# aehogan/lammps-induced-dipole-polarization-pair-style

Measured on AMD Instinct MI355X. Metric: atom-steps/sec, higher is better.
Workload: dtype f64

## Files before the change

### lammps-induced-dipole-polarization-pair-style_amd/csrc/polar_api.hip

```cpp
#include "polar_handle.hpp"

namespace {
void upload_types(polar_handle *h, int ntypes, const double *const t[7]) {
  need_device(h);
  const size_t m = (size_t)(ntypes + 1) * (ntypes + 1);
  std::vector<double> pack(8 * m, 0.0);
  for (size_t k = 0; k < m; k++) {
    pack[8 * k + 0] = t[6][k]; pack[8 * k + 1] = t[5][k]; pack[8 * k + 2] = t[0][k]; pack[8 * k + 3] = t[1][k];
    pack[8 * k + 4] = t[2][k]; pack[8 * k + 5] = t[3][k]; pack[8 * k + 6] = t[4][k];
  }
  h->d_lj.ensure(8 * m);
  HIPCHECK(hipMemcpy(h->d_lj.p, pack.data(), 8 * m * sizeof(double), hipMemcpyHostToDevice));
  h->P.ntypes = ntypes;
  h->P.ljpack = h->d_lj.p;
  h->ntypes = ntypes;
  h->types_set = true;
}

void upload_coul(polar_handle *h, double g_ewald, double qqrd2e, const double *slj, const double *scoul, int nbits,
                 int mask, int shift, double tabinnersq, const double *const t[8]) {
  need_device(h);
  h->P.g_ewald = g_ewald; h->P.qqrd2e = qqrd2e;
  for (int k = 0; k < 4; k++) { h->P.special_lj[k] = slj[k]; h->P.special_coul[k] = scoul[k]; }
  h->P.ncoultablebits = nbits; h->P.ncoulmask = mask; h->P.ncoulshiftbits = shift; h->P.tabinnersq = tabinnersq;
// ... 141 lines not shown
  int n = polar_device_count();
  if (n <= 0 || device < 0 || device >= n) {
    h->have_device = false;
    h->err = "no usable HIP device";
    return POLAR_OK;
  }
  return guarded(h, [&]() {
    HIPCHECK(hipSetDevice(device));
    HIPCHECK(hipStreamCreate(&h->stream));
    for (auto &e : h->ev) HIPCHECK(hipEventCreate(&e));
    {
      int prio_lo = 0, prio_hi = 0;
      HIPCHECK(hipDeviceGetStreamPriorityRange(&prio_lo, &prio_hi));
      HIPCHECK(hipStreamCreateWithPriority(&h->lj_stream, hipStreamNonBlocking, prio_lo));
    }
    HIPCHECK(hipEventCreate(&h->ev_fork)); HIPCHECK(hipEventCreate(&h->ev_join));
    HIPCHECK(hipEventCreate(&h->ev_lj0)); HIPCHECK(hipEventCreate(&h->ev_lj1));
    HIPCHECK(hipEventCreateWithFlags(&h->ev_dl0, hipEventDisableTiming)); HIPCHECK(hipEventCreateWithFlags(&h->ev_dl1, hipEventDisableTiming));
    HIPCHECK(hipEventCreateWithFlags(&h->ev_mu_ready, hipEventDisableTiming));
    for (auto &e : h->ev_fchunk) HIPCHECK(hipEventCreateWithFlags(&e, hipEventDisableTiming));
    for (auto &e : h->ev_ks) HIPCHECK(hipEventCreate(&e));
    HIPCHECK(hipStreamCreateWithFlags(&h->dl_stream, hipStreamNonBlocking));
    if (getenv("POLAR_NO_OVERLAP")) h->overlap_lj = false;
    if (const char *e = getenv("POLAR_LJ_PERS")) h->lj_pers = atoi(e);
    if (const char *e = getenv("POLAR_LJ_PERS_THREADS")) h->lj_pers_threads = std::max(256, std::min(POLAR_LJ_PERS_THREADS, (atoi(e) / 64) * 64));
    { int ncu = 0; if (hipDeviceGetAttribute(&ncu, hipDeviceAttributeMultiprocessorCount, device) == hipSuccess) h->ncu = ncu; }
    HIPCHECK(hipHostMalloc((void **)&h->h_scal, sizeof(Scal)));
    HIPCHECK(hipHostMalloc((void **)&h->h_flags, 16 * sizeof(int)));
    HIPCHECK(hipHostMalloc((void **)&h->h_ddtot, 64 * 16 * sizeof(unsigned long long)));
    h->d_overflow.ensure(16); h->d_ddtot.ensure(64 * 16);
    h->d_scal.ensure(1);
    h->d_slots.ensure((size_t)POLAR_NSLOT * POLAR_SLOT_STRIDE);
    h->have_device = true;
    return POLAR_OK;
  });
}

int polar_destroy(polar_handle *h) {
  if (!h) return POLAR_OK;
  if (h->have_device) {
    (void)hipSetDevice(h->device);
    (void)hipStreamSynchronize(h->stream);
    if (h->lj_stream) { (void)hipStreamSynchronize(h->lj_stream); (void)hipStreamDestroy(h->lj_stream); }
    for (hipEvent_t e : {h->ev_fork, h->ev_join, h->ev_lj0, h->ev_lj1, h->ev_dl0, h->ev_dl1, h->ev_mu_ready}) if (e) (void)hipEventDestroy(e);
    for (hipEvent_t e : h->ev_ks) if (e) (void)hipEventDestroy(e);
    if (h->dl_stream) (void)hipStreamDestroy(h->dl_stream);
// ... 817 lines not shown
```

### lammps-induced-dipole-polarization-pair-style_amd/csrc/polar_handle.hpp

```cpp
#pragma once
#include <hip/hip_runtime.h>

#include <algorithm>
#include <initializer_list>
#include <utility>
#include <chrono>
#include <cmath>
#include <cstdio>
#include <cstdlib>
#include <exception>
#include <cstring>
#include <numeric>
#include <string>
#include <thread>
#include <mutex>
#include <condition_variable>
#include <functional>
#include <memory>
#include <stdexcept>
#include <unistd.h>
#include <vector>

#include "pair_host.hpp"
#include "polar_kernels.hpp"
// ... 225 lines not shown
  int un_pitch = 0;
  int un_lds = 0;
  long long pitch16 = 0;
  int tile_max_u = 0;
  bool tile_reported = false;
  double dens = 0.0;
  std::vector<TileLaunch> tile_launches;
  TileLaunch tile_all{};
  size_t tile_lds_attr[16] = {0, 0, 0, 0, 0, 0, 0, 0, 0, 0, 0, 0, 0, 0, 0, 0};
  size_t tile_build_lds_attr = 0;
  int tile_waves = 4;
  int tile_wide = 0;
  int tile_sw[3] = {2, 2, 2};
  int deterministic = 0;
  Scal *h_scal = nullptr;
  hipEvent_t ev[8] = {};
  hipStream_t lj_stream = nullptr;
  hipEvent_t ev_fork = nullptr, ev_join = nullptr, ev_lj0 = nullptr, ev_lj1 = nullptr, ev_dl0 = nullptr, ev_dl1 = nullptr;
  hipStream_t dl_stream = nullptr;
  hipEvent_t ev_mu_ready = nullptr;
  double *early_mu = nullptr, *early_ef = nullptr, *user_mu = nullptr, *user_ef = nullptr;
  hipEvent_t ev_fchunk[4] = {nullptr, nullptr, nullptr, nullptr};
  bool overlap_lj = true;
  bool lj_forked = false;
  std::vector<double> h_tmp;
  double *h_stage = nullptr;
  DBuf<double> d_trace;
  DBuf<double4> d_ew_kv; DBuf<int4> d_ew_hkl, d_ew_rows;
  DBuf<double2> d_ew_s, d_ew_m, d_ew_part;
  DBuf<double> d_ew_erec, d_ew_vpart, d_ew_out;
  std::vector<double> ew_key;
  int ew_nk = 0, ew_nrow = 0, ew_nm = 0;
  double ew_cell[6] = {0, 0, 0, 0, 0, 0};
  hipEvent_t ev_ks[4] = {nullptr, nullptr, nullptr, nullptr};
  int ntrace = 0;
  size_t h_stage_cap = 0;
};
inline int fail(polar_handle *h, int code, const std::string &m) {
  if (h) h->err = m;
  return code;
}

template <typename F>
int guarded(polar_handle *h, F &&fn) {
  if (!h) return POLAR_ERR_STATE;
  try {
// ... 123 lines not shown
inline bool look_at_state(const polar_handle *h, int sw, int every, int step = 1) {
  const int done_sweeps = sw + 1;
  const int pred = h->last_sweeps;
  if (pred <= 0) return (sw % every) == every - 1;
  if (done_sweeps < pred) return (done_sweeps % 16) == 0;
  const int past = done_sweeps - pred;
  if (past <= 4 * step) return (past % step) == 0;
  return (past % every) == 0;
}
inline bool tile_mode(const polar_handle *h) { return h->ph.st.dd_cutoff > 0.0 && h->sweep_kernel == 4; }
inline MuView mu_view(const polar_handle *h) {
  if (tile_mode(h)) return MuView{reinterpret_cast<char *>(h->d_srec0.p), reinterpret_cast<char *>(h->d_srec1.p), (int)sizeof(SRec)};
  return MuView{reinterpret_cast<char *>(h->d_rec0.p), reinterpret_cast<char *>(h->d_rec1.p), (int)sizeof(AtomRec)};
}
inline const int *own_rows(const polar_handle *h) { return (h->sorted && sharded(h)) ? h->d_ownrows.p : nullptr; }

struct TileUnavailable : std::runtime_error {
  explicit TileUnavailable(const std::string &m) : std::runtime_error(m) {}
};

void launch_scan(long long n, const int *in, long long *out, DBuf<long long> &tot, hipStream_t s);
void build_cells(polar_handle *h);
void compute_slots(polar_handle *h);
void build_lists(polar_handle *h);
void launch_rank_pass(polar_handle *h, bool allpairs, int pass);
void prepare_lp(polar_handle *h);
void sweep_once(polar_handle *h, bool ap);
void sweep_phase(polar_handle *h, int color, int part);
void read_scal(polar_handle *h);
void debug_trace(polar_handle *h, int sw, bool jacobi);
bool accel_begin(polar_handle *h, bool ap);
void accel_export(polar_handle *h, double *dev_local_dots);
void accel_step(polar_handle *h, const double *global_dots);
void accel_export_fused(polar_handle *h, double *ared);
void accel_decide_mix(polar_handle *h, const double *ared, bool diff_first);
void solve(polar_handle *h, bool ap, polar_result *out);
void phase_begin(polar_handle *h, int eflag, int vflag, const double *mu_host);
int phase_finish(polar_handle *h, polar_result *out);
void clear_flags(polar_handle *h);
void tile_fallback(polar_handle *h);
bool grow_pitches(polar_handle *h);
int do_compute(polar_handle *h, int eflag, int vflag, const double *mu_host, polar_result *out);
void step_begin_lists(polar_handle *h, int eflag, int vflag);
bool step_needs_colors(const polar_handle *h);
void step_begin_finish(polar_handle *h);
void build_cluster_lists(polar_handle *h);
void ensure_colors(polar_handle *h);
// ... 9 lines not shown
```

### lammps-induced-dipole-polarization-pair-style_amd/csrc/polar_lists.hpp

```cpp
#pragma once

#include "polar_common.hpp"

namespace polar {

struct CellGrid {
  int trim;
  int nc[3];
  double lo[3], inv[3];
};

__device__ __forceinline__ int cell_of(const CellGrid &g, const Box &b, double x, double y, double z) {
  int c[3];
  double fr3[3];
  frac_coords(b, g.lo, x, y, z, fr3);
#pragma unroll
  for (int k = 0; k < 3; k++) {
    double fr = fr3[k];
    fr -= floor(fr);
    int ck = (int)(fr * g.nc[k]);
    c[k] = ck >= g.nc[k] ? g.nc[k] - 1 : ck;
  }
  return (c[2] * g.nc[1] + c[1]) * g.nc[0] + c[0];
}

// ... 423 lines not shown
                                  const int *__restrict__ sub, int nsub) {
  const long long c = blockIdx.x * (long long)blockDim.x + threadIdx.x;
  if (c >= ncell) return;
  const int a = (int)cell_first[c], e = a + npol[c];
  for (int q = 0; q < nclass; q++) {
    int k = 0;
    for (int j = a; j < e; j++) k += color_class(j, color_s, perm, own_lo, own_hi, sub, nsub) == q;
    cnt[(size_t)q * ncell + c] = k;
  }
}
static __global__ void k_color_fill(long long ncell, int nclass, const long long *__restrict__ cell_first, const int *__restrict__ npol,
                             const int *__restrict__ color_s, const int *__restrict__ perm, const long long *__restrict__ off,
                             int *__restrict__ rows_orig, int own_lo, int own_hi, const int *__restrict__ sub, int nsub) {
  const long long c = blockIdx.x * (long long)blockDim.x + threadIdx.x;
  if (c >= ncell) return;
  const int a = (int)cell_first[c], e = a + npol[c];
  for (int q = 0; q < nclass; q++) {
    long long w = off[(size_t)q * ncell + c];
    for (int j = a; j < e; j++) if (color_class(j, color_s, perm, own_lo, own_hi, sub, nsub) == q) rows_orig[w++] = perm[j];
  }
}

template <bool TRI, bool RECHECK>
static __global__ __launch_bounds__(POLAR_BLOCK) void k_nl_build(const int *__restrict__ rows, int nrows,
                                                          const double4 *__restrict__ pos4, Box box, CellGrid g,
                                                          const long long *__restrict__ cell_first, double cutallsq,
                                                          double ddcutsq, long long nl_pitch, long long dd_pitch,
                                                          int *__restrict__ nl_cnt, int *__restrict__ dd_cnt,
                                                          int *__restrict__ nl_j, int *__restrict__ dd_j,
                                                          double *__restrict__ dd_r2, int pad_dd,
                                                          int dd_shift_qm, int dd_pad_index, int *__restrict__ dd_wrap,
                                                          const int *__restrict__ color_s, double colordistsq,
                                                          int *__restrict__ color_conflict,
                                                          const int *__restrict__ dd_slot,
                                                          int *__restrict__ overflow,
                                                          unsigned long long *__restrict__ dd_total) {
  const int dd_shift = dd_shift_qm & 255, dd_qm = dd_shift_qm >> 8;
  const int lane = threadIdx.x & 63;
  const int row = blockIdx.x * POLAR_ROWS_PER_BLOCK + (threadIdx.x >> 6);
  if (row >= nrows) return;
  const int i = rows ? rows[row] : row;
  const double4 ri = pos4[i];
  const int imol = __double2hiint(ri.w), ipol = __double2loint(ri.w);
  const int icol = (RECHECK && color_s && ipol) ? color_s[i] : -2;
  bool clash = RECHECK && color_s && ipol && icol < 0;
  int cc[3];
  double uu[3], edge[3];
  {
    double fr3[3];
    frac_coords(box, g.lo, ri.x, ri.y, ri.z, fr3);
#pragma unroll
    for (int k = 0; k < 3; k++) {
      double fr = fr3[k];
      fr -= floor(fr);
      const double t = fr * g.nc[k];
      int ck = (int)t;
      ck = ck >= g.nc[k] ? g.nc[k] - 1 : ck;
      cc[k] = __builtin_amdgcn_readfirstlane(ck);
      uu[k] = wave_uniform(t - ck); edge[k] = wave_uniform(box.prd[k] / g.nc[k]);
    }
  }
  const int c0 = cc[0], c1 = cc[1], c2 = cc[2];
  const int slot_i = dd_slot ? dd_slot[i] : i;
// ... 65 lines not shown
          if (dd_r2) dd_r2[dd0 + kd] = rsq;
        }
        ncount += __popcll(m_nl);
        dcount += __popcll(m_dd);
      }
    }
  }
  if (pad_dd) {
    const int have = dcount < dd_pitch ? dcount : (int)dd_pitch;
    const int padded = (have + 63) & ~63;
    for (int k = have + lane; k < padded; k += 64) {
      dd_j[dd0 + (dd_shift ? lp_slot(k, dd_qm) : (long long)k)] = (dd_pad_index >= 0 ? dd_pad_index : i) << dd_shift;
      if (dd_r2) dd_r2[dd0 + k] = 1e60;
    }
  }
  if (RECHECK && color_s && __ballot(clash) != 0ull && lane == 0) atomicOr(color_conflict, 1);
  const unsigned long long anywrap = __ballot(wrap_lane);
  if (lane == 0) {
    nl_cnt[i] = ncount; dd_cnt[i] = dcount;
    if (dd_wrap) dd_wrap[i] = anywrap != 0ull;
    if (ncount > nl_pitch || dcount > dd_pitch) atomicMax(overflow, ncount > dcount ? ncount : dcount);
    if (dcount) atomicAdd(dd_total + (blockIdx.x & 63) * 16, (unsigned long long)(dcount < dd_pitch ? dcount : (int)dd_pitch));
  }
}

#ifdef POLAR_LAB
#include "lab/lists_paired_rows.hpp"
#endif

#ifdef POLAR_LAB
#include "lab/lists_cluster_rows.hpp"
#endif

struct LJGrid {
  int nc[3];
  double lo[3], inv[3];
};
__device__ __forceinline__ int lj_cell_of(const LJGrid &g, double x, double y, double z) {
  const double p[3] = {x, y, z};
  int c[3];
#pragma unroll
  for (int k = 0; k < 3; k++) {
    int ck = (int)floor((p[k] - g.lo[k]) * g.inv[k]);
    c[k] = ck < 0 ? 0 : (ck >= g.nc[k] ? g.nc[k] - 1 : ck);
  }
  return (c[2] * g.nc[1] + c[1]) * g.nc[0] + c[0];
// ... 227 lines not shown
```

### lammps-induced-dipole-polarization-pair-style_amd/csrc/polar_rows.hpp

```cpp
#pragma once

#include "polar_common.hpp"
#include "polar_force_pair.hpp"
#ifdef POLAR_LAB
#include "lab/force_pair_literal.hpp"
#define POLAR_LIT_PARAM , int literal
#define POLAR_LIT_PASS , literal
#else
#define POLAR_LIT_PARAM
#define POLAR_LIT_PASS
#endif

namespace polar {

static __global__ void k_pack(int n, const int *__restrict__ perm, const double *__restrict__ x, const double *__restrict__ q,
                       const double *__restrict__ alpha, const int *__restrict__ mol, const double *__restrict__ mu0,
                       AtomRec *__restrict__ r0, AtomRec *__restrict__ r1, int *__restrict__ mol_s,
                       double4 *__restrict__ pos4, double4 *__restrict__ xq_s, int wrap, Box box, double lo0, double lo1,
                       double lo2) {
  int i = blockIdx.x * blockDim.x + threadIdx.x;
  if (i == n) {
    AtomRec d;
    d.x = n > 0 ? x[0] : 0.0; d.y = n > 0 ? x[1] : 0.0; d.z = n > 0 ? x[2] : 0.0;
    d.mx = d.my = d.mz = d.q = d.a = 0.0;
// ... 337 lines not shown
  double4 *ctab_lds = reinterpret_cast<double4 *>(lj_lds + nlj);
  for (int t = threadIdx.x; t < w * w * 8; t += blockDim.x) lj_lds[t] = P.ljpack[t];
  const int ntable = 1 << P.ncoultablebits;
  for (int b = threadIdx.x; b < ntable; b += blockDim.x) {
    const double2 *bin = reinterpret_cast<const double2 *>(P.ctab + (size_t)b * 8);
    const double2 fdf = bin[1], ede = bin[2];
    ctab_lds[b] = make_double4(fdf.x, fdf.y, ede.x, ede.y);
  }
  __syncthreads();
  const int lane = threadIdx.x & 63, wv = threadIdx.x >> 6, nwv = blockDim.x >> 6;
  double ev = 0.0, ec = 0.0;
  for (int ii = blockIdx.x + gridDim.x * wv; ii < inum; ii += gridDim.x * nwv) {
    const int i = ilist ? ilist[ii] : ii;
    const int jnum = numneigh ? numneigh[i] : (int)(first[i + 1] - first[i]);
    if (jnum == 0) continue;
    double v[6] = {0, 0, 0, 0, 0, 0};
    ljcoul_row<EFLAG, VPAIR, TAB>(P, i, jnum, neigh + first[i], xq[i], xq, type, lj_lds, ctab_lds, lane, f, eatom, vatom, ev, ec, v);
    if (VPAIR) ljcoul_tally<false, true>(slots, ii, lane, vglobal, 0.0, 0.0, v);
  }
  const double none[6] = {0, 0, 0, 0, 0, 0};
  ljcoul_tally<EFLAG, false>(slots, blockIdx.x * nwv + wv, lane, 0, ev, ec, none);
}

template <bool ALLPAIRS, bool EW>
static __device__ __forceinline__ void static_field_body(const int *__restrict__ rows, int nrows, int nlocal,
                                                              const AtomRec *__restrict__ rec,
                                                              const int *__restrict__ mol, Box box,
                                                              RowList nl,
                                                              const int *__restrict__ nl_j, double cut_coulsq,
                                                              double e2s, double gamma, int use_previous,
                                                              double *__restrict__ ef, AtomRec *__restrict__ rec0,
                                                              AtomRec *__restrict__ rec1, const double4 *__restrict__ xq_s,
                                                              double g_ewald, const double *__restrict__ erec) {
  const int lane = threadIdx.x & 63;
  const int row = blockIdx.x * POLAR_ROWS_PER_BLOCK + (threadIdx.x >> 6);
  if (row >= nrows) return;
  const int i = rows ? rows[row] : row;
  const AtomRec ri = uniform_rec(rec[i]);
  const int mi = mol[i];
  const double f_shift = -1.0 / cut_coulsq;
  double ex = 0, ey = 0, ez = 0;
  long long beg = 0, end = nlocal;
  if (!ALLPAIRS) row_range(nl, i, beg, end);
  if (ALLPAIRS) {
    for (long long p = beg + lane; p < end; p += 64) {
      const int j = (int)p;
      if (j == i) continue;
      const AtomRec rj = rec[j];
      double dx, dy, dz;
      pair_del<ALLPAIRS>(box, ri.x, ri.y, ri.z, rj.x, rj.y, rj.z, dx, dy, dz);
      const double rsq = dx * dx + dy * dy + dz * dz;
      if (EW) {
        if (rsq <= cut_coulsq) {
          const double ef_temp = ewald_b1(rsq, g_ewald, (mi != mol[j]) || mi == 0) * rj.q;
          ex += ef_temp * dx; ey += ef_temp * dy; ez += ef_temp * dz;
        }
      } else if (rsq <= cut_coulsq && ((mi != mol[j]) || mi == 0)) {
        const double rinv = rsqrt(rsq);
        const double ef_temp = (rinv * rinv + f_shift) * rinv * rj.q;
        ex += ef_temp * dx; ey += ef_temp * dy; ez += ef_temp * dz;
      }
    }
  } else {
    __shared__ double2 s_stage[POLAR_ROWS_PER_BLOCK][64 * 5];
    double2 *stage = s_stage[threadIdx.x >> 6];
    for (long long base = beg; base < end; base += 64) {
      const long long p = base + lane;
      const bool valid = p < end;
      const int e = valid ? nl_j[p] : i;
      const int j = e & POLAR_NL_MASK;
      double xj, yj, zj, qj;
      if (xq_s) { const XQ t = fetch_xq(xq_s, j, stage, lane); xj = t.a.x; yj = t.a.y; zj = t.b.x; qj = t.b.y; }
      else { const RecQuad rj = fetch_records(rec, j, stage, lane); xj = rj.a.x; yj = rj.b.x; zj = rj.c.x; qj = rj.d.x; }
      double dx, dy, dz;
      pair_del<ALLPAIRS>(box, ri.x, ri.y, ri.z, xj, yj, zj, dx, dy, dz);
      const double rsq = dx * dx + dy * dy + dz * dz;
      if (EW) {
        if (valid && j != i && rsq <= cut_coulsq) {
          const double ef_temp = ewald_b1(rsq, g_ewald, !(e & POLAR_NL_SAMEMOL)) * qj;
          ex += ef_temp * dx; ey += ef_temp * dy; ez += ef_temp * dz;
        }
      } else if (valid && j != i && rsq <= cut_coulsq && !(e & POLAR_NL_SAMEMOL)) {
        const double rinv = rsqrt(rsq);
        const double ef_temp = (rinv * rinv + f_shift) * rinv * qj;
        ex += ef_temp * dx; ey += ef_temp * dy; ez += ef_temp * dz;
      }
    }
  }
  ex = wave_sum(ex); ey = wave_sum(ey); ez = wave_sum(ez);
  if (lane == 0) {
    ex *= e2s; ey *= e2s; ez *= e2s;
    if (EW) { ex += erec[3 * i]; ey += erec[3 * i + 1]; ez += erec[3 * i + 2]; }
    ef[3 * i] = ex; ef[3 * i + 1] = ey; ef[3 * i + 2] = ez;
    if (!use_previous) {
      const double a = ri.a;
      double mx = a * ex, my = a * ey, mz = a * ez;
      mx *= gamma; my *= gamma; mz *= gamma;
      rec0[i].mx = mx; rec0[i].my = my; rec0[i].mz = mz;
      rec1[i].mx = mx; rec1[i].my = my; rec1[i].mz = mz;
    }
  }
}

template <bool ALLPAIRS>
static __global__ __launch_bounds__(POLAR_BLOCK) void k_static_field(const int *__restrict__ rows, int nrows, int nlocal,
                                                              const AtomRec *__restrict__ rec,
                                                              const int *__restrict__ mol, Box box,
                                                              RowList nl,
                                                              const int *__restrict__ nl_j, double cut_coulsq,
                                                              double e2s, double gamma, int use_previous,
                                                              double *__restrict__ ef, AtomRec *__restrict__ rec0,
                                                              AtomRec *__restrict__ rec1, const double4 *__restrict__ xq_s) {
  static_field_body<ALLPAIRS, false>(rows, nrows, nlocal, rec, mol, box, nl, nl_j, cut_coulsq, e2s, gamma, use_previous, ef, rec0, rec1,
                                     xq_s, 0.0, nullptr);
}
template <bool ALLPAIRS>
static __global__ __launch_bounds__(POLAR_BLOCK) void k_ew_static_field(const int *__restrict__ rows, int nrows, int nlocal,
                                                                 const AtomRec *__restrict__ rec,
                                                                 const int *__restrict__ mol, Box box,
                                                                 RowList nl,
                                                                 const int *__restrict__ nl_j, double cut_coulsq,
                                                                 double e2s, double gamma, int use_previous,
                                                                 double *__restrict__ ef, AtomRec *__restrict__ rec0,
                                                                 AtomRec *__restrict__ rec1, const double4 *__restrict__ xq_s,
// ... 160 lines not shown
```

### lammps-induced-dipole-polarization-pair-style_amd/csrc/polar_step.hip

```cpp
#include "polar_handle.hpp"

void launch_scan(long long n, const int *in, long long *out, DBuf<long long> &tot, hipStream_t s) {
  const int nb = (int)std::max<long long>(1, (n + POLAR_SCAN_ITEMS - 1) / POLAR_SCAN_ITEMS);
  tot.ensure((size_t)nb + 1);
  k_scan_block<<<nb, 1024, 0, s>>>(n, in, out, tot.p);
  if (nb > 1) {
    k_scan_totals<<<1, 1024, 0, s>>>(nb, tot.p, out + n);
    k_scan_add<<<nblk(n - POLAR_SCAN_ITEMS, 256), 256, 0, s>>>(n, out, tot.p);
  }
}

void build_cells(polar_handle *h) {
  const polar_settings &st = h->ph.st;
  const int n = h->nlocal;
  const double cutall = std::max(st.cut_coul, st.dd_cutoff);
  double width[3];
  box_widths(h->box, width);
  for (int k = 0; k < 3; k++)
    if (h->box.periodic[k] && width[k] < 2.0 * cutall * (1.0 - 1e-12))
      throw InputError("dd_cutoff mode needs box lengths >= 2*max(cut_coul,dd_cutoff); use exact mode (dd_cutoff 0)");
  CellGrid &g = h->grid;
  g.trim = 1;
#ifdef POLAR_LAB
  if (const char *e = getenv("POLAR_NL_TRIM")) g.trim = atoi(e);
// ... 46 lines not shown
    h->d_ownrows.ensure(own_n(h) + 1);
    k_map_range<<<nblk(own_n(h), 256), 256, 0, s>>>(own_lo(h), own_n(h), h->d_inv.p, h->d_ownrows.p);
  }
}

void compute_slots(polar_handle *h) {
  const polar_settings &st = h->ph.st;
  const bool gs = st.polar_gs || st.polar_gs_ranked;
  const int n = h->nlocal;
  hipStream_t s = h->stream;
  h->d_slot.ensure(n + 1);
  HIPCHECK(hipMemsetAsync(h->d_slot.p, 0xFF, (size_t)(n + 1) * sizeof(int), s));
  if (gs && h->colors_valid) {
    const int tot = h->color_off.empty() ? 0 : h->color_off.back();
    if (tot > 0) k_slot_from_rows<<<nblk(tot, 256), 256, 0, s>>>(tot, h->d_rows.p, h->d_slot.p);
    h->slots_by_color = true;
    h->slots_epoch = h->color_epoch;
  } else {
    k_slot_from_rows<<<nblk(own_n(h), 256), 256, 0, s>>>(own_n(h), own_rows(h), h->d_slot.p);
    h->slots_by_color = false;
  }
}

void build_lists(polar_handle *h) {
  const polar_settings &st = h->ph.st;
  const int n = h->nlocal;
  const double cutall = std::max(st.cut_coul, st.dd_cutoff);
  hipStream_t s = h->stream;
  const CellGrid &g = h->grid;
  if (h->nl_pitch == 0 && getenv("POLAR_INIT_PITCH")) h->nl_pitch = h->dd_pitch = ((std::max(64, atoi(getenv("POLAR_INIT_PITCH"))) + 63) / 64) * 64;
  if (h->nl_pitch == 0) {
    double vol = h->box.prd[0] * h->box.prd[1] * h->box.prd[2];
    {
      int nc[3];
      long long tot = 1;
      for (int k = 0; k < 3; k++) { nc[k] = std::max(1, std::min(64, (int)(h->box.prd[k] / cutall))); tot *= nc[k]; }
      std::vector<char> occ((size_t)tot, 0);
      for (int a = 0; a < n; a++) {
        long long c = 0, mul = 1;
        for (int k = 0; k < 3; k++) {
          double fr = (h->hx[3 * (size_t)a + k] - h->grid.lo[k]) / h->box.prd[k];
          fr -= std::floor(fr);
          c += mul * std::min(nc[k] - 1, (int)(fr * nc[k]));
          mul *= nc[k];
        }
        occ[(size_t)c] = 1;
      }
// ... 23 lines not shown
  h->stream_mode = mode;
  const bool r2c = mode == 1;
  if (mode == 1) h->d_dd_r2.ensure((size_t)n * h->dd_pitch + 64);
  else if (mode == 0) h->d_dd_s.ensure((size_t)n * h->dd_pitch + 64);
  double *r2p = r2c ? h->d_dd_r2.p : nullptr;
  double2 *sp = mode == 0 ? h->d_dd_s.p : nullptr;
  bool fuse = mode != 0 && mode != 4;
#ifdef POLAR_LAB
  if (getenv("POLAR_NO_FUSE_R2")) fuse = false;
#endif
  const double cutallsq = cutall * cutall, ddsq = mode == 4 ? -1.0 : st.dd_cutoff * st.dd_cutoff;
  const int nr = own_n(h);
  const int *rows = own_rows(h);
  zero_many(s, {{h->d_nl_cnt.p, (size_t)(n + 1) * sizeof(int)}, {h->d_dd_cnt.p, (size_t)(n + 1) * sizeof(int)},
                {h->d_overflow.p, 16 * sizeof(int)}, {h->d_ddtot.p, 64 * 16 * sizeof(unsigned long long)}});
  const bool lp = mode == 3;
  if (lp) h->d_dd_wrap.ensure(n + 1);
  const bool recheck = h->colors_valid && h->colors_recheck && h->sweep_kernel < 3 && (int)h->h_color.size() == n;
  if (h->colors_recheck && !recheck) { h->colors_valid = false; h->colors_recheck = false; }
  if (recheck) {
    h->d_color_s.ensure(n + 1);
    k_color_map<<<nblk(n, 256), 256, 0, s>>>(n, h->d_perm.p, h->d_color_orig.p, h->d_color_s.p);
  }
#define NLB(TRI, RC)                                                                                                          \
  k_nl_build<TRI, RC><<<nblk(nr, POLAR_ROWS_PER_BLOCK), POLAR_BLOCK, 0, s>>>(                                                 \
      rows, nr, h->d_pos4.p, h->box, g, h->d_cell_first.p, cutallsq, ddsq, h->nl_pitch, h->dd_pitch, h->d_nl_cnt.p,            \
      h->d_dd_cnt.p, h->d_nl_j.p, h->d_dd_j.p, fuse ? r2p : nullptr, fuse ? 1 : 0, lp ? (6 | (h->lp_quad_major << 8)) : 0,    \
      lp ? n : -1, lp ? h->d_dd_wrap.p : nullptr, recheck ? h->d_color_s.p : nullptr, h->color_keep * h->color_keep,           \
      h->d_overflow.p + 8, lp ? h->d_slot.p : nullptr, h->d_overflow.p, h->d_ddtot.p)
  if (h->box.triclinic) { if (recheck) NLB(true, true); else NLB(true, false); }
  else                  { if (recheck) NLB(false, true); else NLB(false, false); }
#undef NLB
  const RowList ddl{h->d_dd_cnt.p, h->dd_pitch};
  if (fuse || mode == 4) {
  }
#ifdef POLAR_LAB
  else if (st.damping_type == POLAR_DAMP_EXPONENTIAL)
    k_dd_scalars<0><<<nblk(nr, POLAR_ROWS_PER_BLOCK), POLAR_BLOCK, 0, s>>>(rows, nr, h->d_rec0.p, h->box, ddl, h->d_dd_j.p, st.polar_damp, sp, r2p);
  else
    k_dd_scalars<1><<<nblk(nr, POLAR_ROWS_PER_BLOCK), POLAR_BLOCK, 0, s>>>(rows, nr, h->d_rec0.p, h->box, ddl, h->d_dd_j.p, st.polar_damp, sp, r2p);
#endif
  HIPCHECK(hipMemcpyAsync(h->h_flags, h->d_overflow.p, sizeof(int), hipMemcpyDeviceToHost, s));
  HIPCHECK(hipMemcpyAsync(h->h_ddtot, h->d_ddtot.p, 64 * 16 * sizeof(unsigned long long), hipMemcpyDeviceToHost, s));
}
template <bool AP>
static void launch_rank(polar_handle *h, int pass) {
  const int n = h->nlocal, ntot = h->nlocal + h->nghost;
  dim3 grid(nblk(n, POLAR_ROWS_PER_BLOCK)), block(POLAR_BLOCK);
  if (pass == 2) k_fold_scal<<<1, POLAR_NSLOT, 0, h->stream>>>(h->d_scal.p, h->d_slots.p, 1);
  const int nchunk = (AP && pass == 1) ? std::max(1, std::min(16, 8192 / std::max(n, 1))) : 1;
  if (pass == 1)
    k_rank<AP, 1><<<nblk((long long)n * nchunk, POLAR_ROWS_PER_BLOCK), block, 0, h->stream>>>(n, ntot, h->d_x.p, h->d_alpha.p, h->d_mol.p, h->box, RowList{h->d_nl_cnt.p, h->nl_pitch},
                                                 h->d_nl_j.p, h->d_rec0.p, h->d_mol_s.p, h->d_scal.p, h->d_slots.p, h->d_rank.p, nchunk);
  else
    k_rank<AP, 2><<<grid, block, 0, h->stream>>>(n, ntot, h->d_x.p, h->d_alpha.p, h->d_mol.p, h->box, RowList{h->d_nl_cnt.p, h->nl_pitch},
// ... 384 lines not shown
  if (!global_dots)
    k_accel_diff<POLAR_ACCEL_MAXM><<<nb, 256, 0, h->stream>>>(tot, h->acc_pitch, h->d_lpdesc.p, h->d_rec0.p, h->d_scal.p, h->d_acc_state.p, h->d_acc_x.p,
                                                             h->d_acc_f.p, h->d_acc_g.p, h->d_acc_dF.p, h->d_acc_dG.p, h->d_acc_part.p, ring);
  k_accel_solve<POLAR_ACCEL_MAXM><<<1, 256, 0, h->stream>>>(nb, h->d_acc_part.p, h->d_scal.p, h->d_acc_state.p, nullptr, global_dots, ring);
  k_accel_mix<POLAR_ACCEL_MAXM><<<nb, 256, 0, h->stream>>>(tot, h->acc_pitch, h->d_lpdesc.p, h->d_rec0.p, h->d_scal.p, h->d_acc_state.p, h->d_acc_x.p,
                                                          h->d_acc_g.p, h->d_acc_dG.p);
}

void solve(polar_handle *h, bool ap, polar_result *out) {
  const polar_settings &st = h->ph.st;
  const int n = h->nlocal;
  hipStream_t s = h->stream;
  const bool gs = st.polar_gs || st.polar_gs_ranked;
  const bool expd = st.damping_type == POLAR_DAMP_EXPONENTIAL;
  const int max_sweeps = st.iterations_max + 1;
  const int check_every = 4;
  out->ncolors = 0;
  if (st.polar_accel > 0 && (ap || !gs)) throw InputError("polar_accel needs the Gauss-Seidel sweep of list mode (dd_cutoff > 0 with polar_gs or polar_gs_ranked)");

  if (!gs || !ap) {
    const bool clm = !ap && h->sweep_kernel == 3, tile = !ap && h->sweep_kernel == 4;
    if (!ap && !tile) resolve_colors(h);
    if (!tile && (gs || clm) && !h->colors_valid) { ensure_colors(h); if (clm) build_cluster_lists(h); else map_color_rows(h); }
    if (!ap && gs && h->sweep_kernel == 2 && !slots_current(h)) { compute_slots(h); build_lists(h); }
    if (gs) out->ncolors = tile ? (int)h->tile_launches.size() : (int)h->color_off.size() - 1;
    if (!ap && h->sweep_kernel == 2) prepare_lp(h);
#ifdef POLAR_LAB
    if (!ap && h->sweep_kernel == 2 && h->lp_pairs && !deterministic(h)) build_units(h);
#endif
    const bool lazy = st.fixed_iteration && gs;
    const bool accel = accel_begin(h, ap);
    for (int sw = 0; sw < max_sweeps; sw++) {
      sweep_once(h, ap);
      debug_trace(h, sw, !gs);
      if (accel && lazy && sw < max_sweeps - 1) accel_step(h, nullptr);
      if (lazy && sw < max_sweeps - 2) continue;
      const int count = (lazy && sw == max_sweeps - 2) ? max_sweeps - 1 : 1;
      if (accel && !lazy) accel_decide_mix(h, nullptr, true);
      else k_solver_step<<<1, POLAR_NSLOT, 0, s>>>(h->d_scal.p, h->d_slots.p, norm_count(h), st.fixed_iteration, st.iterations_max, st.polar_precision, gs ? 0 : 1, nullptr, count, det_part(h), det_npart(h));
      if (!st.fixed_iteration && look_at_state(h, sw, check_every)) {
        read_scal(h);
        if (h->h_scal->done) break;
      }
    }
  } else if (h->dense_gs) {
    const long long np = ((long long)n + 63) / 64 * 64;
    h->d_T6.ensure((size_t)n * 6 * np + 64);
// ... 199 lines not shown
    }
  }
  h->sorted = false;
  h->dense_gs = false;
  const bool gs_mode = (st.polar_gs || st.polar_gs_ranked) && !st.zodid;
  bool ranked_done = false;
  if (ap && gs_mode && n > 64 && 48.0 * (double)n * (double)n <= 3.2e10 && !getenv("POLAR_NO_DENSE_GS")) {
    h->dense_gs = true;
    if (st.polar_gs_ranked) {
      launch_rank<true>(h, 1); launch_rank<true>(h, 2);
      ranked_done = true;
      h->d_perm.ensure(n + 1); h->d_inv.ensure(n + 1);
      k_rank_order<<<nblk(n, POLAR_ROWS_PER_BLOCK), POLAR_BLOCK, 0, s>>>(n, h->d_rank.p, h->d_perm.p, h->d_inv.p);
      h->sorted = true;
    }
  }
  if (!ap) { build_cells(h); h->d_pos4.ensure(n + 1); if (h->static_xq) h->d_xq_s.ensure(n + 2); }
  k_pack<<<nblk(n + 1, 256), 256, 0, s>>>(n, h->sorted ? h->d_perm.p : nullptr, h->d_x.p, h->d_q.p, h->d_alpha.p, h->d_mol.p, mu0,
                                      h->d_rec0.p, h->d_rec1.p, h->d_mol_s.p, ap ? nullptr : h->d_pos4.p, (!ap && h->static_xq) ? h->d_xq_s.p : nullptr,
                                      (!ap && h->sweep_kernel == 4) ? 1 : 0, h->box, h->boxlo[0], h->boxlo[1], h->boxlo[2]);
  if (!ap) {
    if (h->colors_valid && h->sweep_kernel < 3) map_color_rows(h);
    if (h->sweep_kernel == 2) compute_slots(h);
    build_lists(h);
    if (h->colors_valid && h->sweep_kernel == 3) build_cluster_lists(h);
    if (h->sweep_kernel == 4) build_tiles(h);
  }
  HIPCHECK(hipEventRecord(h->ev[1], s));

  if (st.polar_gs_ranked && (ap || (!h->colors_valid && h->sweep_kernel != 4)) && !ranked_done) {
    if (ap) { launch_rank<true>(h, 1); launch_rank<true>(h, 2); }
    else    { launch_rank<false>(h, 1); launch_rank<false>(h, 2); }
  }
  HIPCHECK(hipEventRecord(h->ev[2], s));

  HIPCHECK(hipEventRecord(h->ev[3], s));

  {
    dim3 grid(nblk(own_n(h), POLAR_ROWS_PER_BLOCK)), block(POLAR_BLOCK);
    const double ccs = st.cut_coul * st.cut_coul, e2s = std::sqrt(h->P.qqrd2e);
    if (ewald_on(h)) {
      ewald_field(h);
      const double g = h->P.g_ewald;
      if (ap) k_ew_static_field<true><<<grid, block, 0, s>>>(nullptr, n, n, h->d_rec0.p, h->d_mol_s.p, h->box, RowList{nullptr, 0}, nullptr, ccs, e2s, st.polar_gamma, st.use_previous, h->d_ef_s.p, h->d_rec0.p, h->d_rec1.p, nullptr, g, h->d_ew_erec.p);
      else    k_ew_static_field<false><<<grid, block, 0, s>>>(own_rows(h), own_n(h), n, h->d_rec0.p, h->d_mol_s.p, h->box, RowList{h->d_nl_cnt.p, h->nl_pitch}, h->d_nl_j.p, ccs, e2s, st.polar_gamma, st.use_previous, h->d_ef_s.p, h->d_rec0.p, h->d_rec1.p, h->static_xq ? h->d_xq_s.p : nullptr, g, h->d_ew_erec.p);
    } else if (ap) k_static_field<true><<<grid, block, 0, s>>>(nullptr, n, n, h->d_rec0.p, h->d_mol_s.p, h->box, RowList{nullptr, 0}, nullptr, ccs, e2s, st.polar_gamma, st.use_previous, h->d_ef_s.p, h->d_rec0.p, h->d_rec1.p, nullptr);
    else    k_static_field<false><<<grid, block, 0, s>>>(own_rows(h), own_n(h), n, h->d_rec0.p, h->d_mol_s.p, h->box, RowList{h->d_nl_cnt.p, h->nl_pitch}, h->d_nl_j.p, ccs, e2s, st.polar_gamma, st.use_previous, h->d_ef_s.p, h->d_rec0.p, h->d_rec1.p, h->static_xq ? h->d_xq_s.p : nullptr);
  }
#ifdef POLAR_LAB
  if (!ap && h->sweep_kernel == 4 && !st.zodid)
    k_srec_pack<<<nblk(n, 256), 256, 0, s>>>(n, h->d_rec0.p, h->d_srec0.p, h->d_srec1.p);
#endif
  HIPCHECK(hipEventRecord(h->ev[4], s));
  if (lj_late) launch_lj();
}

int phase_finish(polar_handle *h, polar_result *out) {
  const polar_settings &st = h->ph.st;
  const int n = h->nlocal, nall = h->nlocal + h->nghost;
  const bool ap = !(st.dd_cutoff > 0.0);
  const bool expd = st.damping_type == POLAR_DAMP_EXPONENTIAL;
  const int eflag = h->step_eflag, vmode = h->step_vflag % 4;
  hipStream_t s = h->stream;
#ifdef POLAR_LAB
  if (!ap && h->sweep_kernel == 4 && !st.zodid)
    k_srec_unpack<<<nblk(n, 256), 256, 0, s>>>(n, h->d_scal.p, h->d_srec0.p, h->d_srec1.p, h->d_rec0.p, h->d_rec1.p);
#endif
  k_fallback<<<nblk(n, 256), 256, 0, s>>>(n, h->d_scal.p, h->d_rec0.p, h->d_rec1.p, h->d_ef_s.p);
// ... 144 lines not shown
  return rc;
}

void step_begin_lists(polar_handle *h, int eflag, int vflag) {
  HIPCHECK(hipSetDevice(h->device));
  clear_flags(h);
  try {
    phase_begin(h, eflag, vflag, nullptr);
  } catch (const TileUnavailable &) {
    tile_fallback(h);
    phase_begin(h, eflag, vflag, nullptr);
  }
  if (h->ph.st.dd_cutoff > 0.0 && !tile_mode(h)) resolve_colors(h);
}
bool step_needs_colors(const polar_handle *h) {
  const polar_settings &st = h->ph.st;
  const bool clm = st.dd_cutoff > 0.0 && h->sweep_kernel == 3;
  return st.dd_cutoff > 0.0 && !tile_mode(h) && !st.zodid && (st.polar_gs || st.polar_gs_ranked || clm) && !h->colors_valid;
}
void step_begin_finish(polar_handle *h) {
  const polar_settings &st = h->ph.st;
  const bool clm = st.dd_cutoff > 0.0 && h->sweep_kernel == 3;
  if (step_needs_colors(h)) { ensure_colors(h); if (clm) build_cluster_lists(h); else map_color_rows(h); }
  if (!st.zodid && st.dd_cutoff > 0.0 && (st.polar_gs || st.polar_gs_ranked) && h->sweep_kernel == 2 && !slots_current(h)) { compute_slots(h); build_lists(h); }
  if (!st.zodid && st.dd_cutoff > 0.0 && h->sweep_kernel == 2) prepare_lp(h);
  h->in_step = true;
}
```

Measured before the change: 16.26 million.

## Fuse static field computation into neighbor list build kernel

Adds a variant of the neighbor list build kernel that computes each row's static electric field and initial dipoles right after writing that row's neighbor list. This drops the separate static-field kernel when sweep_kernel is 2, the xq staging buffer exists and Ewald is off, and it reuses the just-written list entries while they are likely still in cache. The shared per-row loop and finish logic are split into helper functions. In exchange the fused kernel uses more registers and shared memory, which could lower the list builder's occupancy. It also relies on a wave-level fence between the writes and reads of the list.

After: 15.97 million. -1.8%, worse.

```diff
diff --git a/lammps-induced-dipole-polarization-pair-style_amd/csrc/polar_api.hip b/lammps-induced-dipole-polarization-pair-style_amd/csrc/polar_api.hip
--- a/lammps-induced-dipole-polarization-pair-style_amd/csrc/polar_api.hip
+++ b/lammps-induced-dipole-polarization-pair-style_amd/csrc/polar_api.hip
@@ -187,6 +187,7 @@
     for (auto &e : h->ev_ks) HIPCHECK(hipEventCreate(&e));
     HIPCHECK(hipStreamCreateWithFlags(&h->dl_stream, hipStreamNonBlocking));
     if (getenv("POLAR_NO_OVERLAP")) h->overlap_lj = false;
+    if (const char *e = getenv("POLAR_NO_FUSE_STATIC")) h->fuse_static = atoi(e) == 0;
     if (const char *e = getenv("POLAR_LJ_PERS")) h->lj_pers = atoi(e);
     if (const char *e = getenv("POLAR_LJ_PERS_THREADS")) h->lj_pers_threads = std::max(256, std::min(POLAR_LJ_PERS_THREADS, (atoi(e) / 64) * 64));
     { int ncu = 0; if (hipDeviceGetAttribute(&ncu, hipDeviceAttributeMultiprocessorCount, device) == hipSuccess) h->ncu = ncu; }
diff --git a/lammps-induced-dipole-polarization-pair-style_amd/csrc/polar_handle.hpp b/lammps-induced-dipole-polarization-pair-style_amd/csrc/polar_handle.hpp
--- a/lammps-induced-dipole-polarization-pair-style_amd/csrc/polar_handle.hpp
+++ b/lammps-induced-dipole-polarization-pair-style_amd/csrc/polar_handle.hpp
@@ -271,6 +271,7 @@
   double *early_mu = nullptr, *early_ef = nullptr, *user_mu = nullptr, *user_ef = nullptr;
   hipEvent_t ev_fchunk[4] = {nullptr, nullptr, nullptr, nullptr};
   bool overlap_lj = true;
+  bool fuse_static = true;
   bool lj_forked = false;
   std::vector<double> h_tmp;
   double *h_stage = nullptr;
@@ -440,7 +441,8 @@
 void launch_scan(long long n, const int *in, long long *out, DBuf<long long> &tot, hipStream_t s);
 void build_cells(polar_handle *h);
 void compute_slots(polar_handle *h);
-void build_lists(polar_handle *h);
+bool fused_static(const polar_handle *h);
+void build_lists(polar_handle *h, bool with_static);
 void launch_rank_pass(polar_handle *h, bool allpairs, int pass);
 void prepare_lp(polar_handle *h);
 void sweep_once(polar_handle *h, bool ap);
diff --git a/lammps-induced-dipole-polarization-pair-style_amd/csrc/polar_lists.hpp b/lammps-induced-dipole-polarization-pair-style_amd/csrc/polar_lists.hpp
--- a/lammps-induced-dipole-polarization-pair-style_amd/csrc/polar_lists.hpp
+++ b/lammps-induced-dipole-polarization-pair-style_amd/csrc/polar_lists.hpp
@@ -1,6 +1,7 @@
 #pragma once
 
 #include "polar_common.hpp"
+#include "polar_rows.hpp"
 
 namespace polar {
 
@@ -470,23 +471,20 @@
 }
 
 template <bool TRI, bool RECHECK>
-static __global__ __launch_bounds__(POLAR_BLOCK) void k_nl_build(const int *__restrict__ rows, int nrows,
-                                                          const double4 *__restrict__ pos4, Box box, CellGrid g,
-                                                          const long long *__restrict__ cell_first, double cutallsq,
-                                                          double ddcutsq, long long nl_pitch, long long dd_pitch,
-                                                          int *__restrict__ nl_cnt, int *__restrict__ dd_cnt,
-                                                          int *__restrict__ nl_j, int *__restrict__ dd_j,
-                                                          double *__restrict__ dd_r2, int pad_dd,
-                                                          int dd_shift_qm, int dd_pad_index, int *__restrict__ dd_wrap,
-                                                          const int *__restrict__ color_s, double colordistsq,
-                                                          int *__restrict__ color_conflict,
-                                                          const int *__restrict__ dd_slot,
-                                                          int *__restrict__ overflow,
-                                                          unsigned long long *__restrict__ dd_total) {
+static __device__ __forceinline__ bool nl_build_row(const int *__restrict__ rows, int nrows, const double4 *__restrict__ pos4,
+                                                    const Box &box, const CellGrid &g, const long long *__restrict__ cell_first,
+                                                    double cutallsq, double ddcutsq, long long nl_pitch, long long dd_pitch,
+                                                    int *__restrict__ nl_cnt, int *__restrict__ dd_cnt, int *__restrict__ nl_j,
+                                                    int *__restrict__ dd_j, double *__restrict__ dd_r2, int pad_dd,
+                                                    int dd_shift_qm, int dd_pad_index, int *__restrict__ dd_wrap,
+                                                    const int *__restrict__ color_s, double colordistsq,
+                                                    int *__restrict__ color_conflict, const int *__restrict__ dd_slot,
+                                                    int *__restrict__ overflow, unsigned long long *__restrict__ dd_total,
+                                                    int &i_out, double4 &ri_out, int &ncount_out) {
   const int dd_shift = dd_shift_qm & 255, dd_qm = dd_shift_qm >> 8;
   const int lane = threadIdx.x & 63;
   const int row = blockIdx.x * POLAR_ROWS_PER_BLOCK + (threadIdx.x >> 6);
-  if (row >= nrows) return;
+  if (row >= nrows) return false;
   const int i = rows ? rows[row] : row;
   const double4 ri = pos4[i];
   const int imol = __double2hiint(ri.w), ipol = __double2loint(ri.w);
@@ -598,6 +596,70 @@
     if (ncount > nl_pitch || dcount > dd_pitch) atomicMax(overflow, ncount > dcount ? ncount : dcount);
     if (dcount) atomicAdd(dd_total + (blockIdx.x & 63) * 16, (unsigned long long)(dcount < dd_pitch ? dcount : (int)dd_pitch));
   }
+  i_out = i; ri_out = ri; ncount_out = ncount;
+  return true;
+}
+
+template <bool TRI, bool RECHECK>
+static __global__ __launch_bounds__(POLAR_BLOCK) void k_nl_build(const int *__restrict__ rows, int nrows,
+                                                          const double4 *__restrict__ pos4, Box box, CellGrid g,
+                                                          const long long *__restrict__ cell_first, double cutallsq,
+                                                          double ddcutsq, long long nl_pitch, long long dd_pitch,
+                                                          int *__restrict__ nl_cnt, int *__restrict__ dd_cnt,
+                                                          int *__restrict__ nl_j, int *__restrict__ dd_j,
+                                                          double *__restrict__ dd_r2, int pad_dd,
+                                                          int dd_shift_qm, int dd_pad_index, int *__restrict__ dd_wrap,
+                                                          const int *__restrict__ color_s, double colordistsq,
+                                                          int *__restrict__ color_conflict,
+                                                          const int *__restrict__ dd_slot,
+                                                          int *__restrict__ overflow,
+                                                          unsigned long long *__restrict__ dd_total) {
+  int i, ncount;
+  double4 ri;
+  nl_build_row<TRI, RECHECK>(rows, nrows, pos4, box, g, cell_first, cutallsq, ddcutsq, nl_pitch, dd_pitch, nl_cnt, dd_cnt,
+                             nl_j, dd_j, dd_r2, pad_dd, dd_shift_qm, dd_pad_index, dd_wrap, color_s, colordistsq,
+                             color_conflict, dd_slot, overflow, dd_total, i, ri, ncount);
+}
+
+struct StaticTail {
+  double cut_coulsq, e2s, gamma;
+  int use_previous;
+  double *ef;
+  AtomRec *rec0, *rec1;
+  const double4 *xq_s;
+};
+template <bool TRI, bool RECHECK>
+static __global__ __launch_bounds__(POLAR_BLOCK) void k_nl_build_static(const int *__restrict__ rows, int nrows,
+                                                          const double4 *__restrict__ pos4, Box box, CellGrid g,
+                                                          const long long *__restrict__ cell_first, double cutallsq,
+                                                          double ddcutsq, long long nl_pitch, long long dd_pitch,
+                                                          int *__restrict__ nl_cnt, int *__restrict__ dd_cnt,
+                                                          int *__restrict__ nl_j, int *__restrict__ dd_j,
+                                                          double *__restrict__ dd_r2, int pad_dd,
+                                                          int dd_shift_qm, int dd_pad_index, int *__restrict__ dd_wrap,
+                                                          const int *__restrict__ color_s, double colordistsq,
+                                                          int *__restrict__ color_conflict,
+                                                          const int *__restrict__ dd_slot,
+                                                          int *__restrict__ overflow,
+                                                          unsigned long long *__restrict__ dd_total,
+                                                          StaticTail st) {
+  __shared__ double2 s_stage[POLAR_ROWS_PER_BLOCK][64 * 3];
+  int i, ncount;
+  double4 ri;
+  if (!nl_build_row<TRI, RECHECK>(rows, nrows, pos4, box, g, cell_first, cutallsq, ddcutsq, nl_pitch, dd_pitch, nl_cnt,
+                                  dd_cnt, nl_j, dd_j, dd_r2, pad_dd, dd_shift_qm, dd_pad_index, dd_wrap, color_s,
+                                  colordistsq, color_conflict, dd_slot, overflow, dd_total, i, ri, ncount)) return;
+  __builtin_amdgcn_fence(__ATOMIC_RELEASE, "workgroup");
+  __builtin_amdgcn_wave_barrier();
+  __builtin_amdgcn_fence(__ATOMIC_ACQUIRE, "workgroup");
+  const int lane = threadIdx.x & 63;
+  const long long beg = (long long)i * nl_pitch, end = beg + (ncount < nl_pitch ? ncount : nl_pitch);
+  const double xi = wave_uniform(ri.x), yi = wave_uniform(ri.y), zi = wave_uniform(ri.z);
+  const double ai = wave_uniform(st.rec0[i].a);
+  double ex = 0, ey = 0, ez = 0;
+  static_field_list_row<false, true>(i, xi, yi, zi, box, nl_j, beg, end, st.cut_coulsq, nullptr, st.xq_s, s_stage[threadIdx.x >> 6],
+                                     lane, 0.0, ex, ey, ez);
+  static_field_finish<false>(i, lane, ai, ex, ey, ez, st.e2s, st.gamma, st.use_previous, st.ef, st.rec0, st.rec1, nullptr);
 }
 
 #ifdef POLAR_LAB
diff --git a/lammps-induced-dipole-polarization-pair-style_amd/csrc/polar_rows.hpp b/lammps-induced-dipole-polarization-pair-style_amd/csrc/polar_rows.hpp
--- a/lammps-induced-dipole-polarization-pair-style_amd/csrc/polar_rows.hpp
+++ b/lammps-induced-dipole-polarization-pair-style_amd/csrc/polar_rows.hpp
@@ -383,6 +383,56 @@
   ljcoul_tally<EFLAG, false>(slots, blockIdx.x * nwv + wv, lane, 0, ev, ec, none);
 }
 
+template <bool EW, bool XQ_ONLY>
+static __device__ __forceinline__ void static_field_list_row(int i, double xi, double yi, double zi, const Box &box, const int *nl_j,
+                                                             long long beg, long long end, double cut_coulsq,
+                                                             const AtomRec *__restrict__ rec, const double4 *__restrict__ xq_s,
+                                                             double2 *stage, int lane, double g_ewald, double &ex, double &ey,
+                                                             double &ez) {
+  const double f_shift = -1.0 / cut_coulsq;
+  for (long long base = beg; base < end; base += 64) {
+    const long long p = base + lane;
+    const bool valid = p < end;
+    const int e = valid ? nl_j[p] : i;
+    const int j = e & POLAR_NL_MASK;
+    double xj, yj, zj, qj;
+    if (XQ_ONLY || xq_s) { const XQ t = fetch_xq(xq_s, j, stage, lane); xj = t.a.x; yj = t.a.y; zj = t.b.x; qj = t.b.y; }
+    else { const RecQuad rj = fetch_records(rec, j, stage, lane); xj = rj.a.x; yj = rj.b.x; zj = rj.c.x; qj = rj.d.x; }
+    double dx, dy, dz;
+    pair_del<false>(box, xi, yi, zi, xj, yj, zj, dx, dy, dz);
+    const double rsq = dx * dx + dy * dy + dz * dz;
+    if (EW) {
+      if (valid && j != i && rsq <= cut_coulsq) {
+        const double ef_temp = ewald_b1(rsq, g_ewald, !(e & POLAR_NL_SAMEMOL)) * qj;
+        ex += ef_temp * dx; ey += ef_temp * dy; ez += ef_temp * dz;
+      }
+    } else if (valid && j != i && rsq <= cut_coulsq && !(e & POLAR_NL_SAMEMOL)) {
+      const double rinv = rsqrt(rsq);
+      const double ef_temp = (rinv * rinv + f_shift) * rinv * qj;
+      ex += ef_temp * dx; ey += ef_temp * dy; ez += ef_temp * dz;
+    }
+  }
+}
+template <bool EW>
+static __device__ __forceinline__ void static_field_finish(int i, int lane, double alpha, double ex, double ey, double ez, double e2s,
+                                                           double gamma, int use_previous, double *__restrict__ ef,
+                                                           AtomRec *__restrict__ rec0, AtomRec *__restrict__ rec1,
+                                                           const double *__restrict__ erec) {
+  ex = wave_sum(ex); ey = wave_sum(ey); ez = wave_sum(ez);
+  if (lane == 0) {
+    ex *= e2s; ey *= e2s; ez *= e2s;
+    if (EW) { ex += erec[3 * i]; ey += erec[3 * i + 1]; ez += erec[3 * i + 2]; }
+    ef[3 * i] = ex; ef[3 * i + 1] = ey; ef[3 * i + 2] = ez;
+    if (!use_previous) {
+      const double a = alpha;
+      double mx = a * ex, my = a * ey, mz = a * ez;
+      mx *= gamma; my *= gamma; mz *= gamma;
+      rec0[i].mx = mx; rec0[i].my = my; rec0[i].mz = mz;
+      rec1[i].mx = mx; rec1[i].my = my; rec1[i].mz = mz;
+    }
+  }
+}
+
 template <bool ALLPAIRS, bool EW>
 static __device__ __forceinline__ void static_field_body(const int *__restrict__ rows, int nrows, int nlocal,
                                                               const AtomRec *__restrict__ rec,
@@ -424,43 +474,10 @@
     }
   } else {
     __shared__ double2 s_stage[POLAR_ROWS_PER_BLOCK][64 * 5];
-    double2 *stage = s_stage[threadIdx.x >> 6];
-    for (long long base = beg; base < end; base += 64) {
-      const long long p = base + lane;
-      const bool valid = p < end;
-      const int e = valid ? nl_j[p] : i;
-      const int j = e & POLAR_NL_MASK;
-      double xj, yj, zj, qj;
-      if (xq_s) { const XQ t = fetch_xq(xq_s, j, stage, lane); xj = t.a.x; yj = t.a.y; zj = t.b.x; qj = t.b.y; }
-      else { const RecQuad rj = fetch_records(rec, j, stage, lane); xj = rj.a.x; yj = rj.b.x; zj = rj.c.x; qj = rj.d.x; }
-      double dx, dy, dz;
-      pair_del<ALLPAIRS>(box, ri.x, ri.y, ri.z, xj, yj, zj, dx, dy, dz);
-      const double rsq = dx * dx + dy * dy + dz * dz;
-      if (EW) {
-        if (valid && j != i && rsq <= cut_coulsq) {
-          const double ef_temp = ewald_b1(rsq, g_ewald, !(e & POLAR_NL_SAMEMOL)) * qj;
-          ex += ef_temp * dx; ey += ef_temp * dy; ez += ef_temp * dz;
-        }
-      } else if (valid && j != i && rsq <= cut_coulsq && !(e & POLAR_NL_SAMEMOL)) {
-        const double rinv = rsqrt(rsq);
-        const double ef_temp = (rinv * rinv + f_shift) * rinv * qj;
-        ex += ef_temp * dx; ey += ef_temp * dy; ez += ef_temp * dz;
-      }
-    }
-  }
-  ex = wave_sum(ex); ey = wave_sum(ey); ez = wave_sum(ez);
-  if (lane == 0) {
-    ex *= e2s; ey *= e2s; ez *= e2s;
-    if (EW) { ex += erec[3 * i]; ey += erec[3 * i + 1]; ez += erec[3 * i + 2]; }
-    ef[3 * i] = ex; ef[3 * i + 1] = ey; ef[3 * i + 2] = ez;
-    if (!use_previous) {
-      const double a = ri.a;
-      double mx = a * ex, my = a * ey, mz = a * ez;
-      mx *= gamma; my *= gamma; mz *= gamma;
-      rec0[i].mx = mx; rec0[i].my = my; rec0[i].mz = mz;
-      rec1[i].mx = mx; rec1[i].my = my; rec1[i].mz = mz;
-    }
-  }
+    static_field_list_row<EW, false>(i, ri.x, ri.y, ri.z, box, nl_j, beg, end, cut_coulsq, rec, xq_s, s_stage[threadIdx.x >> 6], lane,
+                                     g_ewald, ex, ey, ez);
+  }
+  static_field_finish<EW>(i, lane, ri.a, ex, ey, ez, e2s, gamma, use_previous, ef, rec0, rec1, erec);
 }
 
 template <bool ALLPAIRS>
diff --git a/lammps-induced-dipole-polarization-pair-style_amd/csrc/polar_step.hip b/lammps-induced-dipole-polarization-pair-style_amd/csrc/polar_step.hip
--- a/lammps-induced-dipole-polarization-pair-style_amd/csrc/polar_step.hip
+++ b/lammps-induced-dipole-polarization-pair-style_amd/csrc/polar_step.hip
@@ -92,7 +92,12 @@
   }
 }
 
-void build_lists(polar_handle *h) {
+bool fused_static(const polar_handle *h) {
+  const polar_settings &st = h->ph.st;
+  return h->fuse_static && st.dd_cutoff > 0.0 && h->sweep_kernel == 2 && h->static_xq && !ewald_on(h);
+}
+
+void build_lists(polar_handle *h, bool with_static) {
   const polar_settings &st = h->ph.st;
   const int n = h->nlocal;
   const double cutall = std::max(st.cut_coul, st.dd_cutoff);
@@ -162,15 +167,22 @@
     h->d_color_s.ensure(n + 1);
     k_color_map<<<nblk(n, 256), 256, 0, s>>>(n, h->d_perm.p, h->d_color_orig.p, h->d_color_s.p);
   }
-#define NLB(TRI, RC)                                                                                                          \
-  k_nl_build<TRI, RC><<<nblk(nr, POLAR_ROWS_PER_BLOCK), POLAR_BLOCK, 0, s>>>(                                                 \
+#define NLB_ARGS                                                                                                              \
       rows, nr, h->d_pos4.p, h->box, g, h->d_cell_first.p, cutallsq, ddsq, h->nl_pitch, h->dd_pitch, h->d_nl_cnt.p,            \
       h->d_dd_cnt.p, h->d_nl_j.p, h->d_dd_j.p, fuse ? r2p : nullptr, fuse ? 1 : 0, lp ? (6 | (h->lp_quad_major << 8)) : 0,    \
       lp ? n : -1, lp ? h->d_dd_wrap.p : nullptr, recheck ? h->d_color_s.p : nullptr, h->color_keep * h->color_keep,           \
-      h->d_overflow.p + 8, lp ? h->d_slot.p : nullptr, h->d_overflow.p, h->d_ddtot.p)
+      h->d_overflow.p + 8, lp ? h->d_slot.p : nullptr, h->d_overflow.p, h->d_ddtot.p
+#define NLB(TRI, RC)                                                                                                          \
+  do {                                                                                                                        \
+    if (with_static) k_nl_build_static<TRI, RC><<<nblk(nr, POLAR_ROWS_PER_BLOCK), POLAR_BLOCK, 0, s>>>(NLB_ARGS, tail);       \
+    else k_nl_build<TRI, RC><<<nblk(nr, POLAR_ROWS_PER_BLOCK), POLAR_BLOCK, 0, s>>>(NLB_ARGS);                                \
+  } while (0)
+  const StaticTail tail{st.cut_coul * st.cut_coul, std::sqrt(h->P.qqrd2e), st.polar_gamma, st.use_previous, h->d_ef_s.p,
+                        h->d_rec0.p, h->d_rec1.p, h->d_xq_s.p};
   if (h->box.triclinic) { if (recheck) NLB(true, true); else NLB(true, false); }
   else                  { if (recheck) NLB(false, true); else NLB(false, false); }
 #undef NLB
+#undef NLB_ARGS
   const RowList ddl{h->d_dd_cnt.p, h->dd_pitch};
   if (fuse || mode == 4) {
   }
@@ -601,7 +613,7 @@
     const bool clm = !ap && h->sweep_kernel == 3, tile = !ap && h->sweep_kernel == 4;
     if (!ap && !tile) resolve_colors(h);
     if (!tile && (gs || clm) && !h->colors_valid) { ensure_colors(h); if (clm) build_cluster_lists(h); else map_color_rows(h); }
-    if (!ap && gs && h->sweep_kernel == 2 && !slots_current(h)) { compute_slots(h); build_lists(h); }
+    if (!ap && gs && h->sweep_kernel == 2 && !slots_current(h)) { compute_slots(h); build_lists(h, false); }
     if (gs) out->ncolors = tile ? (int)h->tile_launches.size() : (int)h->color_off.size() - 1;
     if (!ap && h->sweep_kernel == 2) prepare_lp(h);
 #ifdef POLAR_LAB
@@ -847,7 +859,7 @@
   if (!ap) {
     if (h->colors_valid && h->sweep_kernel < 3) map_color_rows(h);
     if (h->sweep_kernel == 2) compute_slots(h);
-    build_lists(h);
+    build_lists(h, fused_static(h));
     if (h->colors_valid && h->sweep_kernel == 3) build_cluster_lists(h);
     if (h->sweep_kernel == 4) build_tiles(h);
   }
@@ -869,6 +881,7 @@
       const double g = h->P.g_ewald;
       if (ap) k_ew_static_field<true><<<grid, block, 0, s>>>(nullptr, n, n, h->d_rec0.p, h->d_mol_s.p, h->box, RowList{nullptr, 0}, nullptr, ccs, e2s, st.polar_gamma, st.use_previous, h->d_ef_s.p, h->d_rec0.p, h->d_rec1.p, nullptr, g, h->d_ew_erec.p);
       else    k_ew_static_field<false><<<grid, block, 0, s>>>(own_rows(h), own_n(h), n, h->d_rec0.p, h->d_mol_s.p, h->box, RowList{h->d_nl_cnt.p, h->nl_pitch}, h->d_nl_j.p, ccs, e2s, st.polar_gamma, st.use_previous, h->d_ef_s.p, h->d_rec0.p, h->d_rec1.p, h->static_xq ? h->d_xq_s.p : nullptr, g, h->d_ew_erec.p);
+    } else if (fused_static(h)) {
     } else if (ap) k_static_field<true><<<grid, block, 0, s>>>(nullptr, n, n, h->d_rec0.p, h->d_mol_s.p, h->box, RowList{nullptr, 0}, nullptr, ccs, e2s, st.polar_gamma, st.use_previous, h->d_ef_s.p, h->d_rec0.p, h->d_rec1.p, nullptr);
     else    k_static_field<false><<<grid, block, 0, s>>>(own_rows(h), own_n(h), n, h->d_rec0.p, h->d_mol_s.p, h->box, RowList{h->d_nl_cnt.p, h->nl_pitch}, h->d_nl_j.p, ccs, e2s, st.polar_gamma, st.use_previous, h->d_ef_s.p, h->d_rec0.p, h->d_rec1.p, h->static_xq ? h->d_xq_s.p : nullptr);
   }
@@ -1059,7 +1072,7 @@
   const polar_settings &st = h->ph.st;
   const bool clm = st.dd_cutoff > 0.0 && h->sweep_kernel == 3;
   if (step_needs_colors(h)) { ensure_colors(h); if (clm) build_cluster_lists(h); else map_color_rows(h); }
-  if (!st.zodid && st.dd_cutoff > 0.0 && (st.polar_gs || st.polar_gs_ranked) && h->sweep_kernel == 2 && !slots_current(h)) { compute_slots(h); build_lists(h); }
+  if (!st.zodid && st.dd_cutoff > 0.0 && (st.polar_gs || st.polar_gs_ranked) && h->sweep_kernel == 2 && !slots_current(h)) { compute_slots(h); build_lists(h, false); }
   if (!st.zodid && st.dd_cutoff > 0.0 && h->sweep_kernel == 2) prepare_lp(h);
   h->in_step = true;
 }
```
